# gau-nernst/llama-x

Measured on AMD Instinct MI355X. Metric: train tokens/sec Llama-3.1-8B seq4096 at 1/2/4/8 MI355X; p50 step ms, higher is better.
Workload: dtype bf16; 1 GPU; Llama-3.1-8B text-only LoRA r=16 bf16, seq=4096, 1 sequence per GPU, causal mask, base+LM head frozen (BASELINE.json configs[1]); random-init weights at 8B dimensions; seq_len=4096, parallelism=dp1, launch=hipGraph replay (fwd+bwd+AdamW), lm_head_rows=labelled only

## Files before the change

### include/llx.h

```cpp
#ifndef LLX_H
#define LLX_H

#include <stdint.h>

#ifdef __cplusplus
extern "C" {
#endif

typedef void* llx_stream_t;

int llx_version(void);
const char* llx_last_error_string(void);
int llx_device_info(int device, char* name, int len);

int llx_rmsnorm_fwd(const void* x, const void* w, void* y, float* rstd, int64_t rows, int64_t dim, float eps, llx_stream_t s);
int llx_rmsnorm_fwd_quant(const void* x, const void* w, void* y, float* rstd, void* q, int64_t ldq, void* qscale, int64_t rows, int64_t dim,
                          float eps, llx_stream_t s);
int64_t llx_rmsnorm_bwd_workspace_bytes(int64_t rows, int64_t dim);
int llx_rmsnorm_bwd(const void* dy, const void* x, const void* w, const float* rstd, void* dx, void* dw ,
                    int dw_accumulate, void* workspace, const void* dres ,
                    int64_t rows, int64_t dim, llx_stream_t s);

int llx_gemm_nt_bf16(const void* A, int64_t lda, const void* B, int64_t ldb, void* C, int64_t ldc, int64_t M, int64_t N, int64_t K,
                     const void* A2, int64_t lda2, const void* B2, int64_t ldb2, int64_t K2, int epilogue, const void* E, int64_t lde,
                     llx_stream_t s);
int llx_gemm_nt_bf16_rows(const void* A, int64_t lda, const void* B, int64_t ldb, void* C, int64_t ldc, int64_t M, int64_t N, int64_t K,
                          const void* A2, int64_t lda2, const void* B2, int64_t ldb2, int64_t K2, int epilogue, const void* E, int64_t lde,
                          const int32_t* m_valid, llx_stream_t s);
int llx_gemm_nt_bf16_splitk(const void* A, int64_t lda, const void* B, int64_t ldb, float* partial, int64_t M, int64_t N, int64_t K, int splits,
                            const int32_t* m_valid, llx_stream_t s);
int llx_splitk_combine(const float* partial, int splits, int64_t M, int64_t N, const int32_t* inv, const float* scale, void* out, int64_t ld_out,
                       llx_stream_t s);
int llx_gemm_nt_bf16_rope(const void* A, int64_t lda, const void* B, int64_t ldb, void* C, int64_t ldc, int64_t M, int64_t N, int64_t K,
                          const void* A2, int64_t lda2, const void* B2, int64_t ldb2, int64_t K2, const float* rope_table, int64_t rope_S,
                          int64_t rope_cols, llx_stream_t s);

int llx_gemm_tn_bf16(const void* A, int64_t lda, const void* B, int64_t ldb, void* C, int64_t ldc, int64_t M, int64_t N1, int64_t N2,
                     llx_stream_t s);
int llx_gemm_tn_bf16_rows(const void* A, int64_t lda, const void* B, int64_t ldb, void* C, int64_t ldc, int64_t M, int64_t N1, int64_t N2,
                          const int32_t* m_valid, llx_stream_t s);
// ... 135 lines not shown
```

### llama-x_amd/csrc/gemm_bf16.hip

```cpp
#include "common.h"
#include <type_traits>
#include <mutex>

#define BM 256
#define BN 256
#define BK 64
#define STAGE_BYTES (2 * 256 * BK * 2)
#define A_TILE_BYTES (256 * BK * 2)
#define EPI_ROW_BYTES 528
#define GEMM_LDS_BYTES (256 * EPI_ROW_BYTES)

enum { EPI_NONE = 0, EPI_RESIDUAL = 1, EPI_BIAS = 2, EPI_BIAS_GELU = 3, EPI_COLSCALE = 4, EPI_ROWCOLSCALE = 5, EPI_SWIGLU_BWD = 6, EPI_SWIGLU_FWD = 7, EPI_ROPE = 8, EPI_SPLITK = 9, EPI_ROWCOLSCALE_F32 = 10 };

struct GemmArgs {
  const bf16_t* A; const bf16_t* B; bf16_t* C;
  const bf16_t* A2; const bf16_t* B2;
  const bf16_t* E;
  const bf16_t* E2;
  int64_t lda, ldb, ldc, lde, lda2, ldb2;
  int M, N, K, K2;
  int grid_m, grid_n;
  int col0, col_end;
  const bf16_t* sa; const bf16_t* sb;
  const float* rope;
  int rope_S, rope_cols;
  const int* m_valid;
  float* C32;
  int splits;
};

typedef __attribute__((address_space(3))) void lds_void;
typedef const __attribute__((address_space(1))) void gbl_void;

__device__ __forceinline__ float gelu_erf(float x) { return 0.5f * x * (1.0f + erff(x * 0.70710678118654752440f)); }

template <int EPI, bool I8, int PIPE, int BNT = 256>
__global__ __launch_bounds__(512, 2) void gemm_nt_kernel(const GemmArgs g) {
  static_assert(BNT == 256 || BNT == 128, "tile width");
  static_assert(PIPE == 1, "the four-phase main loop is the only one");
  static_assert(BNT == 256 || EPI != EPI_SWIGLU_FWD, "the SwiGLU-forward epilogue needs the full tile");
  constexpr int ESZ = I8 ? 1 : 2;
  constexpr int TK = 128 / ESZ;
  constexpr int WNG = BNT / 64;
  constexpr int WR = 256 / (8 / WNG);
  constexpr int MI = WR / 16;
  constexpr int MH = MI / 2;
  constexpr int BSI = BNT / 64;
  constexpr int EROW = BNT * 2 + 16;
  extern __shared__ __attribute__((aligned(16))) char smem[];
  const int tid = threadIdx.x;
  const int lane = tid & 63;
  const int wave = __builtin_amdgcn_readfirstlane(tid >> 6);
  const int wm = wave / WNG, wn = wave % WNG;

  int grid_m = g.grid_m;
// ... 2 lines not shown
  const int nwg = grid_m * g.grid_n * nsplit;
  int bid = blockIdx.x;
  if (bid >= nwg) return;
  {
    const int q = nwg >> 3, r = nwg & 7, x = bid & 7;
    bid = (x < r ? x * (q + 1) : r * (q + 1) + (x - r) * q) + (bid >> 3);
  }
  const int split = EPI == EPI_SPLITK ? bid / (grid_m * g.grid_n) : 0;
  if constexpr (EPI == EPI_SPLITK) bid -= split * (grid_m * g.grid_n);
  const int GROUP_M = 4;
  const int width = GROUP_M * g.grid_n;
  const int group = bid / width;
  const int gsz = min(grid_m - group * GROUP_M, GROUP_M);
  const int pid_m = group * GROUP_M + ((bid % width) % gsz);
  const int pid_n = (bid % width) / gsz;
  constexpr bool SPLITN = EPI == EPI_SWIGLU_FWD;
  const int halfN = g.N >> 1;
  const int m0 = pid_m * BM, n0 = SPLITN ? pid_n * (BN / 2) : g.col0 + pid_n * BNT;
  auto col_of = [&](int nl) { return SPLITN ? (nl < BN / 2 ? n0 + nl : halfN + n0 + nl - BN / 2) : min(n0 + nl, g.col_end - 1); };

  const int srow = tid >> 3;
  const int schunk = (tid & 7) ^ ((tid >> 4) & 7);
  int arow[4], brow[4];
#pragma unroll
  for (int i = 0; i < 4; ++i) {
    arow[i] = min(m0 + i * 64 + srow, g.M - 1);
    brow[i] = SPLITN ? (i < 2 ? n0 + i * 64 + srow : halfN + n0 + (i - 2) * 64 + srow) : min(n0 + (i % BSI) * 64 + srow, g.col_end - 1);
  }
  const int nk1 = g.K / TK / nsplit;
  const int nk = nk1 + g.K2 / 64;
  const int kofs = split * nk1;
// ... 67 lines not shown
#pragma unroll
      for (int mi = 0; mi < MI; ++mi) rsv[mi] = bf2f(g.sa[min(m0 + wm * WR + mi * 16 + frow, g.M - 1)]);
#pragma unroll
      for (int mi = 0; mi < MI; ++mi) {
        const float rs = rsv[mi];
#pragma unroll
        for (int ni = 0; ni < 4; ++ni) {
          f32x4_t cf;
#pragma unroll
          for (int e = 0; e < 4; ++e) cf[e] = bf2f(f2bf(((float)acc[mi][ni][e] * rs) * sbv[ni][e]));
          acc[mi][ni] = __builtin_bit_cast(acc_t, cf);
        }
      }
    }
  };
  stage_q(0, 0); stage_q(0, 1); stage_q(0, 2); stage_q(0, 3);
  stage_q(1, 2); stage_q(1, 3); stage_q(1, 0);
  auto ktile = [&](int kt, auto ext_tag) __attribute__((always_inline)) {
    auto mfma = [&](const i32x4_t& b, const i32x4_t& a, acc_t& c) { mfma_t(ext_tag, b, a, c); };
    const char* sA = smem + (kt & 1) * STAGE_BYTES;
    const char* sB = sA + A_TILE_BYTES;
    if (kt + 1 < nk) {
      if constexpr (BSI == 4) asm volatile("s_waitcnt vmcnt(6)" ::: "memory");
      else asm volatile("s_waitcnt vmcnt(4)" ::: "memory");
    } else asm volatile("s_waitcnt vmcnt(0)" ::: "memory");
    __builtin_amdgcn_s_barrier();
    asm volatile("" ::: "memory");
    stage_q(kt + 1, 1);
    i32x4_t bfr[2][4], af[2 * MH];
#pragma unroll
// ... 154 lines not shown
          for (int e = 0; e < 4; ++e) c[e] = ((float)acc[mi][ni][e] * rs) * sbv[ni][e];
        }
      } else {
#pragma unroll
        for (int e = 0; e < 4; ++e) c[e] = acc[mi][ni][e];
      }
      u32x2_t pk;
      pk[0] = pack_bf2(c[0], c[1]);
      pk[1] = pack_bf2(c[2], c[3]);
      *reinterpret_cast<u32x2_t*>(smem + m * EROW + n * 2) = pk;
    }
  }
  __syncthreads();
  if constexpr (SPLITN) {
    bf16_t* H = const_cast<bf16_t*>(g.E);
#pragma unroll 4
    for (int it = 0; it < 8; ++it) {
      const int q = it * 512 + tid;
      const int row = q >> 4, cc = q & 15;
      const int gm = m0 + row, gn = n0 + cc * 8;
      if (gm < g.M) {
        const u32x4_t gv = *reinterpret_cast<const u32x4_t*>(smem + row * EPI_ROW_BYTES + cc * 16);
        const u32x4_t uv = *reinterpret_cast<const u32x4_t*>(smem + row * EPI_ROW_BYTES + (cc + 16) * 16);
        *reinterpret_cast<u32x4_t*>(g.C + (int64_t)gm * g.ldc + gn) = gv;
        *reinterpret_cast<u32x4_t*>(g.C + (int64_t)gm * g.ldc + halfN + gn) = uv;
        *reinterpret_cast<u32x4_t*>(H + (int64_t)gm * g.lde + gn) = swiglu_fwd8(gv, uv);
      }
    }
    return;
  }
  auto combine = [&](int it0, const u32x4_t (&aux0)[EB], const u32x4_t (&aux1)[EB]) {
#pragma unroll
    for (int j = 0; j < EB; ++j) {
      const int q = (it0 + j) * 512 + tid;
      const int row = q / (BNT / 8), cc = q % (BNT / 8);
      const int gm = m0 + row, gn = n0 + cc * 8;
      if (gm < g.M && gn < g.col_end) {
        u32x4_t v = *reinterpret_cast<const u32x4_t*>(smem + row * EROW + cc * 16);
        if constexpr (EPI == EPI_RESIDUAL) {
          const u32x4_t r = aux0[j];
#pragma unroll
// ... 40 lines not shown
  auto kern = gemm_nt_kernel<EPI, I8, 1, BNT>;
  static std::once_flag attr_once;
  static hipError_t attr_err = hipSuccess;
  std::call_once(attr_once, [&] { attr_err = hipFuncSetAttribute((const void*)kern, hipFuncAttributeMaxDynamicSharedMemorySize, GEMM_LDS_BYTES); });
  if (attr_err != hipSuccess) {
    llx_set_error("llx_gemm_nt_bf16: cannot raise dynamic LDS limit: %s", hipGetErrorString(attr_err));
    return LLX_ERR_LAUNCH;
  }
  hipLaunchKernelGGL(kern, dim3(a.grid_m * a.grid_n * (EPI == EPI_SPLITK ? a.splits : 1)), dim3(512), GEMM_LDS_BYTES, stream, a);
  LLX_LAUNCH_CHECK("llx_gemm_nt_bf16");
  return LLX_OK;
}

template <int EPI, bool I8 = false>
static int launch_gemm(const GemmArgs& a, hipStream_t stream) {
  if constexpr (EPI != EPI_SWIGLU_FWD) {
    const int tiles = a.grid_m * a.grid_n, tail = tiles % 256;
    if (a.col0 == 0 && a.col_end == a.N && a.N % 256 == 0 && tiles > 256 && tail > 0 && tail <= 128 && tail % a.grid_m == 0) {
      const int tail_cols = tail / a.grid_m * 256;
      GemmArgs full = a, half = a;
      full.col_end = a.N - tail_cols;
      full.grid_n = a.grid_n - tail / a.grid_m;
      half.col0 = a.N - tail_cols;
      half.grid_n = tail_cols / 128;
      const int rc = launch_gemm_p<EPI, I8, 256>(full, stream);
      if (rc != LLX_OK) return rc;
      return launch_gemm_p<EPI, I8, 128>(half, stream);
    }
  }
  return launch_gemm_p<EPI, I8>(a, stream);
}
// ... 6 lines not shown
  a.grid_m = (int)cdiv64(M, BM); a.grid_n = (int)cdiv64(N, BN);
  a.col_end = (int)N;
  a.splits = 1;
  return a;
}

static int check_extent(const char* who, int64_t M, int64_t N, int64_t K, int64_t lda, int64_t ldb, int esz) {
  LLX_REQUIRE(M < (1 << 30) && N < (1 << 30) && K < (1 << 30), "%s: dimension too large", who);
  LLX_REQUIRE(M * lda * esz < (int64_t)4294967296 && N * ldb * esz < (int64_t)4294967296, "%s: operand larger than 4 GiB (32-bit tile offsets)", who);
  return LLX_OK;
}

static int gemm_nt_bf16_impl(const void* A, int64_t lda, const void* B, int64_t ldb, void* C, int64_t ldc, int64_t M,
                             int64_t N, int64_t K, const void* A2, int64_t lda2, const void* B2, int64_t ldb2, int64_t K2,
                             int epilogue, const void* E, int64_t lde, const float* rope, int64_t rope_S, int64_t rope_cols,
                             hipStream_t stream, const int32_t* m_valid = nullptr) {
  LLX_REQUIRE(A && B && C, "llx_gemm_nt_bf16: null pointer");
  LLX_REQUIRE(M > 0 && N > 0 && K > 0, "llx_gemm_nt_bf16: empty problem M=%lld N=%lld K=%lld", (long long)M, (long long)N, (long long)K);
  LLX_REQUIRE(K % BK == 0 && K2 % BK == 0, "llx_gemm_nt_bf16: K=%lld and K2=%lld must be multiples of 64", (long long)K, (long long)K2);
  LLX_REQUIRE(N % 8 == 0, "llx_gemm_nt_bf16: N=%lld must be a multiple of 8", (long long)N);
  LLX_REQUIRE(lda % 8 == 0 && ldb % 8 == 0 && ldc % 8 == 0, "llx_gemm_nt_bf16: row strides must be multiples of 8 elements");
  LLX_REQUIRE(((uintptr_t)A | (uintptr_t)B | (uintptr_t)C) % 16 == 0, "llx_gemm_nt_bf16: pointers must be 16-byte aligned");
  LLX_REQUIRE(K2 == 0 || (A2 && B2 && lda2 % 8 == 0 && ldb2 % 8 == 0 && ((uintptr_t)A2 | (uintptr_t)B2) % 16 == 0),
              "llx_gemm_nt_bf16: bad K-extension operands");
  LLX_REQUIRE(epilogue == EPI_NONE || epilogue == EPI_ROPE || (E && (uintptr_t)E % 16 == 0), "llx_gemm_nt_bf16: epilogue operand missing/unaligned");
  LLX_REQUIRE(epilogue != EPI_ROPE || (rope && (uintptr_t)rope % 16 == 0 && rope_S > 0 && rope_cols >= 0 && rope_cols <= N && rope_cols % 128 == 0),
              "llx_gemm_nt_bf16_rope: need an aligned fp32 table, rope_S > 0 and rope_cols a multiple of 128 within N");
  LLX_REQUIRE((epilogue != EPI_RESIDUAL && epilogue != EPI_SWIGLU_BWD) || lde % 8 == 0, "llx_gemm_nt_bf16: residual / gate|up stride must be a multiple of 8");
  LLX_REQUIRE(epilogue != EPI_SWIGLU_BWD || (lde >= 2 * N && ldc >= 2 * N), "llx_gemm_nt_bf16: the SwiGLU-backward epilogue reads E[M,2N] (gate|up) and writes C[M,2N] (dg|du)");
  if (const int rc = check_extent("llx_gemm_nt_bf16", M, N, K, lda, ldb, 2); rc != LLX_OK) return rc;
  GemmArgs a = make_args(A, lda, B, ldb, C, ldc, M, N, K);
  a.A2 = (const bf16_t*)A2; a.B2 = (const bf16_t*)B2; a.lda2 = lda2; a.ldb2 = ldb2; a.K2 = (int)K2;
  a.E = (const bf16_t*)E; a.lde = lde;
  a.rope = rope; a.rope_S = (int)rope_S; a.rope_cols = (int)rope_cols;
  a.m_valid = m_valid;
  switch (epilogue) {
    case EPI_NONE: return launch_gemm<EPI_NONE>(a, stream);
    case EPI_RESIDUAL: return launch_gemm<EPI_RESIDUAL>(a, stream);
    case EPI_BIAS: return launch_gemm<EPI_BIAS>(a, stream);
    case EPI_BIAS_GELU: return launch_gemm<EPI_BIAS_GELU>(a, stream);
    case EPI_COLSCALE: return launch_gemm<EPI_COLSCALE>(a, stream);
    case EPI_SWIGLU_BWD: return launch_gemm<EPI_SWIGLU_BWD>(a, stream);
    case EPI_ROPE: return launch_gemm<EPI_ROPE>(a, stream);
    case EPI_SWIGLU_FWD:
      LLX_REQUIRE(N % 256 == 0 && lde % 8 == 0, "llx_gemm_nt_bf16: the SwiGLU-forward epilogue needs N = 2I with I a multiple of 128");
      a.grid_n = (int)(N / 256);
      return launch_gemm<EPI_SWIGLU_FWD>(a, stream);
    default: llx_set_error("llx_gemm_nt_bf16: unknown epilogue %d", epilogue); return LLX_ERR_UNSUPPORTED;
  }
}

extern "C" int llx_gemm_nt_bf16(const void* A, int64_t lda, const void* B, int64_t ldb, void* C, int64_t ldc, int64_t M,
                                int64_t N, int64_t K, const void* A2, int64_t lda2, const void* B2, int64_t ldb2, int64_t K2,
                                int epilogue, const void* E, int64_t lde, hipStream_t stream) {
  LLX_REQUIRE(epilogue != EPI_ROPE, "llx_gemm_nt_bf16: the RoPE epilogue is llx_gemm_nt_bf16_rope");
  return gemm_nt_bf16_impl(A, lda, B, ldb, C, ldc, M, N, K, A2, lda2, B2, ldb2, K2, epilogue, E, lde, nullptr, 0, 0, stream);
}

extern "C" int llx_gemm_nt_bf16_rows(const void* A, int64_t lda, const void* B, int64_t ldb, void* C, int64_t ldc, int64_t M,
                                     int64_t N, int64_t K, const void* A2, int64_t lda2, const void* B2, int64_t ldb2, int64_t K2,
                                     int epilogue, const void* E, int64_t lde, const int32_t* m_valid, hipStream_t stream) {
  LLX_REQUIRE(epilogue != EPI_ROPE, "llx_gemm_nt_bf16_rows: the RoPE epilogue is llx_gemm_nt_bf16_rope");
  LLX_REQUIRE(m_valid && (uintptr_t)m_valid % 4 == 0, "llx_gemm_nt_bf16_rows: m_valid must be a device int32 pointer");
  return gemm_nt_bf16_impl(A, lda, B, ldb, C, ldc, M, N, K, A2, lda2, B2, ldb2, K2, epilogue, E, lde, nullptr, 0, 0, stream, m_valid);
}

extern "C" int llx_gemm_nt_bf16_splitk(const void* A, int64_t lda, const void* B, int64_t ldb, float* partial, int64_t M, int64_t N,
                                       int64_t K, int splits, const int32_t* m_valid, hipStream_t stream) {
  LLX_REQUIRE(A && B && partial, "llx_gemm_nt_bf16_splitk: null pointer");
  LLX_REQUIRE(M > 0 && N > 0 && K > 0 && splits >= 1 && splits <= 16, "llx_gemm_nt_bf16_splitk: bad sizes");
  LLX_REQUIRE(K % ((int64_t)BK * splits) == 0, "llx_gemm_nt_bf16_splitk: K=%lld must be a multiple of 64 * splits (%d)", (long long)K, splits);
  LLX_REQUIRE(N % 8 == 0 && lda % 8 == 0 && ldb % 8 == 0, "llx_gemm_nt_bf16_splitk: N and the row strides must be multiples of 8");
  LLX_REQUIRE(((uintptr_t)A | (uintptr_t)B | (uintptr_t)partial) % 16 == 0, "llx_gemm_nt_bf16_splitk: pointers must be 16-byte aligned");
  if (const int rc = check_extent("llx_gemm_nt_bf16_splitk", M, N, K, lda, ldb, 2); rc != LLX_OK) return rc;
  LLX_REQUIRE(m_valid == nullptr || (uintptr_t)m_valid % 4 == 0, "llx_gemm_nt_bf16_splitk: m_valid must be a device int32 pointer");
  GemmArgs a = make_args(A, lda, B, ldb, nullptr, N, M, N, K);
  a.m_valid = m_valid;
  a.C32 = partial; a.splits = splits;
  return launch_gemm_p<EPI_SPLITK, false>(a, stream);
// ... 100 lines not shown
```

### llama-x_amd/csrc/skinny.hip

```cpp
#include "common.h"

typedef __attribute__((address_space(3))) s16x4_t lds_s16x4;
typedef __attribute__((ext_vector_type(8))) short s16x8_t;

#define SK_PAD 64

#define SNT_WAVES 8
#define SNT_UNROLL 8

struct SkinnyRanges { int lo[4], hi[4]; };

__device__ __forceinline__ void snt_scaled_store(const bf16x8_t& a, const bf16_t* cs, bf16_t* g) {
  const u32x4_t x = __builtin_bit_cast(u32x4_t, a);
  const u32x4_t c = *reinterpret_cast<const u32x4_t*>(cs);
  u32x4_t o;
#pragma unroll
  for (int e = 0; e < 4; ++e) o[e] = pack_bf2(bflo(x[e]) * bflo(c[e]), bfhi(x[e]) * bfhi(c[e]));
  *reinterpret_cast<u32x4_t*>(g) = o;
}

template <int NB, bool RANGED, bool SCALE = false>
__global__ __launch_bounds__(SNT_WAVES * 64) void skinny_nt_kernel(const bf16_t* __restrict__ X, int64_t ldx, const bf16_t* __restrict__ W,
                                                                   int64_t ldw, bf16_t* __restrict__ out, int M, int K, int R, SkinnyRanges kr,
                                                                   const bf16_t* __restrict__ cs = nullptr, bf16_t* __restrict__ G = nullptr,
// ... 420 lines not shown
    *reinterpret_cast<u32x2_t*>(out + (int64_t)(m0 + threadIdx.x) * SK_PAD + blockIdx.y * 4) = pk;
  }
}

extern "C" int llx_skinny_u_reduce(const void* upart, void* out, int64_t M, int64_t N, int64_t R, const int32_t* segs, int seg_count, hipStream_t stream) {
  LLX_REQUIRE(upart && out && M > 0 && N > 0 && R > 0 && R <= 64, "llx_skinny_u_reduce: bad arguments");
  TnSegs sg;
  int64_t total = 0;
  const int rc = tn_fill_segs(sg, segs, seg_count, N, R, &total);
  if (rc != LLX_OK) return rc;
  hipLaunchKernelGGL(skinny_u_reduce_kernel, dim3((unsigned)cdiv64(M, 64), SK_PAD / 4), dim3(256), 0, stream, (const float*)upart, (bf16_t*)out, (int)M, (int)R, sg);
  LLX_LAUNCH_CHECK("llx_skinny_u_reduce");
  return LLX_OK;
}

struct TnRed { const float* partial; bf16_t* out; int64_t out_ld, total; int nsplit, RP, R, N, transpose_out, accumulate, use_segs; float scale; TnSegs sg; };
struct TnRedMany { TnRed d[TN_MANY]; };

__global__ void skinny_tn_reduce_many_kernel(const TnRedMany m) {
  const TnRed& d = m.d[blockIdx.y];
  int64_t idx = (int64_t)blockIdx.x * blockDim.x + threadIdx.x;
  if (idx >= d.total) return;
  int r, n;
  bf16_t* dst;
  if (d.use_segs) {
    int s = 0;
    for (; s < d.sg.count; ++s) {
      const int64_t cnt = (int64_t)(d.sg.n_hi[s] - d.sg.n_lo[s]) * (d.sg.r_hi[s] - d.sg.r_lo[s]);
      if (idx < cnt) break;
      idx -= cnt;
// ... 193 lines not shown
```

### llama-x_amd/llx/_lib.py

```python
from __future__ import annotations

import ctypes
import os
from ctypes import c_char_p, c_float, c_int, c_int64, c_void_p

import torch

_HERE = os.path.dirname(os.path.abspath(__file__))
LIB_PATH = os.environ.get("LLX_LIB_PATH") or os.path.join(_HERE, "libllx_hip.so")

_lib = None

_P, _I, _L, _F = c_void_p, c_int, c_int64, c_float
SIGNATURES: dict[str, tuple] = {
    "llx_version": (c_int, []),
    "llx_last_error_string": (c_char_p, []),
    "llx_device_info": (c_int, [c_int, c_char_p, c_int]),
    "llx_rmsnorm_fwd": (c_int, [_P, _P, _P, _P, _L, _L, _F, _P]),
    "llx_rmsnorm_fwd_quant": (c_int, [_P, _P, _P, _P, _P, _L, _P, _L, _L, _F, _P]),
    "llx_rmsnorm_bwd_workspace_bytes": (c_int64, [_L, _L]),
    "llx_rmsnorm_bwd": (c_int, [_P, _P, _P, _P, _P, _P, _I, _P, _P, _L, _L, _P]),
    "llx_attn_flags_bytes": (c_int64, [_L, _L]),
    "llx_attn_tile_flags": (c_int, [_P, _P, _P, _L, _L, _P]),
    "llx_attn_fwd": (c_int, [_P, _L, _L, _P, _L, _L, _P, _L, _L, _P, _L, _L, _P, _P, _P, _P, _L, _L, _L, _L, _L, _F, _P]),
# ... 44 lines not shown
    "llx_gather_rows": (c_int, [_P, _L, _P, _P, _P, _L, _L, _L, _P]),
    "llx_scatter_rows": (c_int, [_P, _L, _P, _P, _P, _L, _L, _L, _P]),
    "llx_skinny_nt": (c_int, [_P, _L, _P, _L, _P, _L, _L, _L, _P, _P]),
    "llx_skinny_nt_scaled": (c_int, [_P, _L, _P, _L, _P, _L, _L, _L, _P, _P, _P, _L, _P]),
    "llx_rmsnorm_skinny_nt": (c_int, [_P, _P, _P, _L, _P, _P, _P, _L, _L, _L, _F, _P]),
    "llx_skinny_tn_workspace_bytes": (c_int64, [_L, _L, _L]),
    "llx_skinny_tn": (c_int, [_P, _P, _L, _P, _L, _L, _L, _L, _F, _I, _I, _P, _P, _I, _P]),
    "llx_skinny_tn_partial": (c_int, [_P, _P, _L, _L, _L, _L, _P, _P, _I, _P]),
    "llx_skinny_tn_partial_many": (c_int, [_I, _P, _P, _P, _P, _P, _P, _P, _P, _P, _P]),
    "llx_skinny_u_workspace_bytes": (_L, [_L, _L]),
    "llx_skinny_tn_partial_many_u": (c_int, [_I, _P, _P, _P, _P, _P, _P, _P, _P, _P, _P, _P, _P, _P]),
    "llx_skinny_u_reduce": (c_int, [_P, _P, _L, _L, _L, _P, _I, _P]),
    "llx_skinny_tn_partial_many_us": (c_int, [_I, _P, _P, _P, _P, _P, _P, _P, _P, _P, _P, _P, _P, _P, _P, _P, _P]),
    "llx_skinny_tn_reduce_many": (c_int, [_I, _P, _P, _P, _P, _P, _P, _P, _P, _P, _P, _P, _P]),
    "llx_gemm_nt_bf16": (c_int, [_P, _L, _P, _L, _P, _L, _L, _L, _L, _P, _L, _P, _L, _L, _I, _P, _L, _P]),
    "llx_gemm_nt_bf16_splitk": (c_int, [_P, _L, _P, _L, _P, _L, _L, _L, _I, _P, _P]),
    "llx_splitk_combine": (c_int, [_P, _I, _L, _L, _P, _P, _P, _L, _P]),
    "llx_gemm_nt_bf16_rows": (c_int, [_P, _L, _P, _L, _P, _L, _L, _L, _L, _P, _L, _P, _L, _L, _I, _P, _L, _P, _P]),
    "llx_gemm_tn_bf16": (c_int, [_P, _L, _P, _L, _P, _L, _L, _L, _L, _P]),
    "llx_gemm_tn_bf16_rows": (c_int, [_P, _L, _P, _L, _P, _L, _L, _L, _L, _P, _P]),
    "llx_gemm_nt_bf16_rope": (c_int, [_P, _L, _P, _L, _P, _L, _L, _L, _L, _P, _L, _P, _L, _L, _P, _L, _L, _P]),
}

DEBUG_SIGNATURES: dict[str, tuple] = {
    "llx_debug_attn_fwd_occupancy": (c_int, []),
    "llx_debug_attn_bwd_set_stamps": (c_int, [_P]),
    "llx_debug_attn_fwd_stamps": (c_int, [_P, _P, _P, _P, _L, _L, _L, _P, _P]),
}


# ... 48 lines not shown
```

### llama-x_amd/llx/kernels.py

```python
from __future__ import annotations

import ctypes
import math
import os
from dataclasses import dataclass
from typing import Optional, Sequence

import torch
from torch import Tensor

from . import _lib as L

BF16 = torch.bfloat16
EPI_NONE, EPI_RESIDUAL, EPI_BIAS, EPI_BIAS_GELU, EPI_COLSCALE = 0, 1, 2, 3, 4
EPI_SWIGLU_BWD = 6
EPI_SWIGLU_FWD = 7
SK_PAD = 64
GEMM_TRACE = None
ATTN_TRACE = None


def _lib():
    return L.load()

# ... 66 lines not shown
    dw = ws = None
    if need_dw:
        dw = dw_out if dw_out is not None else torch.empty(dim, device=x.device, dtype=BF16)
        assert dw.shape == (dim,) and dw.is_contiguous() and dw.dtype is BF16
        ws = torch.empty(_lib().llx_rmsnorm_bwd_workspace_bytes(rows, dim), device=x.device, dtype=torch.uint8)
    if dres is not None:
        dres = _rows2d(dres)
        assert dres.shape == x2.shape and dres.stride(0) == dim
    L.check(_lib().llx_rmsnorm_bwd(L.ptr(dy2), L.ptr(x2), L.ptr(w), L.ptr(rstd), L.ptr(dx), L.ptr(dw), 0, L.ptr(ws), L.ptr(dres), rows, dim,
                                   L.stream()), "llx_rmsnorm_bwd")
    return dx.view(x.shape), dw


def gemm_nt(a: Tensor, b: Tensor, *, out: Optional[Tensor] = None, a2: Optional[Tensor] = None, b2: Optional[Tensor] = None,
            epilogue: int = EPI_NONE, e: Optional[Tensor] = None, rope: Optional[tuple[Tensor, int, int]] = None,
            k2_eff: Optional[float] = None, m_valid: Optional[Tensor] = None, m_expect: Optional[float] = None) -> Tensor:
    _chk_bf16(a, b, a2, b2, e, out)
    assert a.dim() == 2 and b.dim() == 2 and a.shape[1] == b.shape[1], (a.shape, b.shape)
    assert a.stride(1) == 1 and b.stride(1) == 1
    M, K = a.shape
    N = b.shape[0]
    if epilogue == EPI_SWIGLU_BWD:
        assert out is not None and e is not None and out.shape == (M, 2 * N) and e.shape == (M, 2 * N) and out.stride(1) == 1 and e.stride(1) == 1
    else:
        if out is None:
            out = torch.empty(M, N, device=a.device, dtype=BF16)
        assert out.shape == (M, N) and out.stride(1) == 1
    K2 = 0
    if a2 is not None:
        assert b2 is not None and a2.shape[0] == M and b2.shape[0] == N and a2.shape[1] == b2.shape[1]
        assert a2.stride(1) == 1 and b2.stride(1) == 1
# ... 1 lines not shown
    lde = 0
    if epilogue == EPI_RESIDUAL:
        assert e is not None and e.shape == (M, N) and e.stride(1) == 1
        lde = e.stride(0)
    elif epilogue == EPI_SWIGLU_BWD:
        lde = e.stride(0)
    elif epilogue == EPI_SWIGLU_FWD:
        assert e is not None and N % 256 == 0 and e.shape == (M, N // 2) and e.stride(1) == 1
        lde = e.stride(0)
    elif epilogue != EPI_NONE:
        assert e is not None and e.shape == (N,) and e.is_contiguous()
    ev = None
    if GEMM_TRACE is not None:
        ev = (torch.cuda.Event(enable_timing=True), torch.cuda.Event(enable_timing=True))
        ev[0].record()
    if rope is not None:
        table, rs, rc = rope
        assert epilogue == EPI_NONE and table.dtype is torch.float32 and table.is_contiguous() and table.shape[0] >= rs and table.shape[1:] == (64, 2)
        L.check(_lib().llx_gemm_nt_bf16_rope(L.ptr(a), a.stride(0), L.ptr(b), b.stride(0), L.ptr(out), out.stride(0), M, N, K,
                                             L.ptr(a2), a2.stride(0) if a2 is not None else 0, L.ptr(b2), b2.stride(0) if b2 is not None else 0, K2,
                                             L.ptr(table), rs, rc, L.stream()), "llx_gemm_nt_bf16_rope")
    elif m_valid is not None:
        assert m_valid.dtype is torch.int32 and m_valid.numel() == 1 and m_valid.device == a.device
        L.check(_lib().llx_gemm_nt_bf16_rows(L.ptr(a), a.stride(0), L.ptr(b), b.stride(0), L.ptr(out), out.stride(0), M, N, K,
                                             L.ptr(a2), a2.stride(0) if a2 is not None else 0, L.ptr(b2), b2.stride(0) if b2 is not None else 0, K2,
                                             epilogue, L.ptr(e), lde, L.ptr(m_valid), L.stream()), "llx_gemm_nt_bf16_rows")
    else:
        L.check(_lib().llx_gemm_nt_bf16(L.ptr(a), a.stride(0), L.ptr(b), b.stride(0), L.ptr(out), out.stride(0), M, N, K,
                                        L.ptr(a2), a2.stride(0) if a2 is not None else 0, L.ptr(b2), b2.stride(0) if b2 is not None else 0, K2,
                                        epilogue, L.ptr(e), lde, L.stream()), "llx_gemm_nt_bf16")
    if ev is not None:
# ... 610 lines not shown
    assert x.dim() == 2 and w.dim() == 2 and x.shape[1] == w.shape[1] and x.stride(1) == 1 and w.stride(1) == 1
    M, K = x.shape
    R = w.shape[0]
    out = torch.empty(M, SK_PAD, device=x.device, dtype=BF16)
    kr = None
    if kranges is not None:
        assert len(kranges) == 8
        kr = (ctypes.c_int32 * 8)(*[int(v) for v in kranges])
    if colscale is not None:
        assert colscale.shape == (K,) and colscale.is_contiguous()
        g = torch.empty(M, K, device=x.device, dtype=BF16)
        L.check(_lib().llx_skinny_nt_scaled(L.ptr(x), x.stride(0), L.ptr(w), w.stride(0), L.ptr(out), M, K, R, kr, L.ptr(colscale), L.ptr(g), K,
                                            L.stream()), "llx_skinny_nt_scaled")
        return out, g
    L.check(_lib().llx_skinny_nt(L.ptr(x), x.stride(0), L.ptr(w), w.stride(0), L.ptr(out), M, K, R, kr, L.stream()), "llx_skinny_nt")
    return out


@dataclass
class TnQueued:
    ws: Tensor
    out: Tensor
    out_ld: int
    M: int
    N: int
    R: int
    scale: float
    transpose_out: int
    accumulate: int
    segs: Optional[ctypes.Array]
# ... 71 lines not shown
```

### llama-x_amd/llx/ops.py

```python
from __future__ import annotations

import os

from typing import Optional, Sequence

import torch
from torch import Tensor, nn
from torch.autograd import Function

from . import kernels as K
from ._lib import LlxError

BF16 = torch.bfloat16


def _cached_multi(tensors: Sequence[Tensor], tag: str, build):
    store = tensors[0].__dict__.setdefault("_llx_cache", {})
    key = tuple((t._version, str(t.device)) for t in tensors)
    hit = store.get(tag)
    if hit is not None and hit[0] == key:
        return hit[1]
    val = build()
    store[tag] = (key, val)
    return val
# ... 181 lines not shown
        if self.int8 and self.dynamic:
            return _cached_multi(ws, "cat_i8", lambda: torch.cat([w.detach() for w in ws], 0))
        if self.int8:
            return _cached_multi(ws, "cat_bf16", lambda: K.i8_to_bf16(torch.cat([w.detach() for w in ws], 0)))
        return _cached_multi(ws, "cat", lambda: torch.cat([w.detach() for w in ws], 0) if len(ws) > 1 else ws[0].detach())

    def wt_cat(self) -> Tensor:
        ws = self._weights()
        return _cached_multi(ws, "cat_t", lambda: K.transpose(torch.cat([w.detach() for w in ws], 0) if len(ws) > 1 else ws[0].detach()))

    def scale_cat(self) -> Tensor:
        ss = [m.weight.scale for m in self.members]
        return _cached_multi(ss, "cat_scale", lambda: torch.cat(ss, 0) if len(ss) > 1 else ss[0])

    def forward(self, x: Tensor, out: Optional[Tensor] = None, residual: Optional[Tensor] = None, swiglu_h: Optional[Tensor] = None,
                rope: Optional[tuple[Tensor, int, int]] = None, xq: Optional[tuple[Tensor, Tensor]] = None, t_pre: Optional[Tensor] = None):
        if out is None:
            out = torch.empty(x.shape[0], self.N, device=x.device, dtype=BF16)
        return out, self._forward(x, out, residual, swiglu_h, rope, xq, t_pre)

    def norm_can_make_t(self, dim: int) -> bool:
        return self.fused and self.R > 0 and self.packed is not None and K.rmsnorm_skinny_ok(dim)

    def wants_quantized_input(self) -> bool:
        return self.fused and self.int8 and self.dynamic

    def rope_fusable(self) -> bool:
        return self.fused and (not self.int8 or self.dynamic) and not self.dora

    def swiglu_fusable(self) -> bool:
        return self.fused and (not self.int8 or self.dynamic) and not self.dora and len(self.members) == 2 and self.Ns[0] % 128 == 0

    def _forward(self, x: Tensor, out: Tensor, residual: Optional[Tensor], swiglu_h: Optional[Tensor] = None,
                 rope: Optional[tuple[Tensor, int, int]] = None, xq: Optional[tuple[Tensor, Tensor]] = None, t_pre: Optional[Tensor] = None):
        if not self.fused:
            assert residual is None or len(self.members) == 1
            return [m.forward(x, out=out[:, o : o + n], residual=residual)[1] for m, o, n in zip(self.members, self.n_off, self.Ns)]
        t = b2 = None
        if self.R > 0:
            a_cat, b2, bT, a2t = self.packed or K.lora_group_pack([m.lora_a.detach() for m in self.members],
                                                                  [m.lora_b.detach() for m in self.members], self.K, self.scale)
            t = (t_pre if t_pre is not None else K.skinny_nt(x, a_cat), bT, a2t)
        if self.dora:
            assert swiglu_h is None and rope is None
            c, inv = dora_colscale(self.members, self.w_cat(), a_cat, b2)
            z = K.gemm_nt(x, self.w_cat(), a2=t[0], b2=b2, k2_eff=self.k2_fwd)
            K.scale(z, colscale=c, out=out)
            if residual is not None:
                K.add(out, residual, out=out)
            return (*t, z, c, inv)
        if not self.int8:
            if residual is not None:
                K.gemm_nt(x, self.w_cat(), out=out, a2=t[0] if t else None, b2=b2, epilogue=K.EPI_RESIDUAL, e=residual, k2_eff=self.k2_fwd)
            elif swiglu_h is not None:
                K.gemm_nt(x, self.w_cat(), out=out, a2=t[0] if t else None, b2=b2, epilogue=K.EPI_SWIGLU_FWD, e=swiglu_h, k2_eff=self.k2_fwd)
            else:
                K.gemm_nt(x, self.w_cat(), out=out, a2=t[0] if t else None, b2=b2, rope=rope, k2_eff=self.k2_fwd)
            return t
        if self.dynamic:
            from subclasses.int8 import quantize_int8_rowwise
            from subclasses.int8_mm import _launch as i8_gemm

            xi, xs = xq if xq is not None else quantize_int8_rowwise(x)
            a2, bb = (t[0], b2) if self.R > 0 else (None, None)
            if residual is not None:
                i8_gemm(xi, self.w_cat(), xs, self.scale_cat(), out=out, a2=a2, b2=bb, epilogue=K.EPI_RESIDUAL, e=residual)
            elif swiglu_h is not None:
                i8_gemm(xi, self.w_cat(), xs, self.scale_cat(), out=out, a2=a2, b2=bb, epilogue=K.EPI_SWIGLU_FWD, e=swiglu_h)
            else:
                i8_gemm(xi, self.w_cat(), xs, self.scale_cat(), out=out, a2=a2, b2=bb, rope=rope)
# ... 324 lines not shown
        return (dx.view(B, S, D) if (dx is not None and need_dx) else None, None, dnw, None, *g_qkv, *g_o)


_HEAD_COMPACT = os.environ.get("LLX_HEAD_COMPACT", "1") != "0"
_HEAD_SPLITK = max(1, int(os.environ.get("LLX_HEAD_SPLITK", "4")))
_HEAD_CHUNK_FORCED = "LLX_HEAD_CHUNK_ROWS" in os.environ
_HEAD_CHUNK_ROWS = max(256, int(os.environ.get("LLX_HEAD_CHUNK_ROWS", "8192")) // 256 * 256)


class MLPBlockMeta:
    def __init__(self, w13: GroupPlan, w2: GroupPlan, eps, fuse_norm, fuse_residual):
        self.w13, self.w2 = w13, w2
        self.eps, self.fuse_norm, self.fuse_residual = eps, fuse_norm, fuse_residual


class MLPBlockFn(Function):
    @staticmethod
    def forward(ctx, x: Tensor, norm_w: Optional[Tensor], meta: MLPBlockMeta, *tensors):
        K.L.require_cuda(x)
        shape = x.shape
        x2 = K._rows2d(x.contiguous())
        xn, rstd, xq, t_pre = _norm_prologue(meta, meta.w13, x2, norm_w)
        T, I = x2.shape[0], meta.w13.Ns[0]
        gu = torch.empty(T, 2 * I, device=x.device, dtype=BF16)
        if meta.w13.swiglu_fusable():
            h = torch.empty(T, I, device=x.device, dtype=BF16)
            _, t13 = meta.w13.forward(xn, gu, swiglu_h=h, xq=xq, t_pre=t_pre)
        else:
            _, t13 = meta.w13.forward(xn, gu, xq=xq, t_pre=t_pre)
            h = K.swiglu_fwd(gu[:, :I], gu[:, I:])
        y, t2 = meta.w2.forward(h, None, x2 if meta.fuse_residual else None)
        ctx.meta = meta
        _save(ctx, x, norm_w, x2, xn if meta.fuse_norm else None, rstd, gu, h, t13, t2)
        return y.view(shape)

    @staticmethod
    def backward(ctx, dy: Tensor):
        meta: MLPBlockMeta = ctx.meta
        x, norm_w, x2, xn, rstd, gu, h, t13, t2 = _load(ctx)
        if xn is None:
            xn = x2
        T, I = x2.shape[0], meta.w13.Ns[0]
        dy2 = K._rows2d(dy.contiguous())
        needs = list(ctx.needs_input_grad[3:])
        n_13 = len(meta.w13.tensors())
        n13, n2 = needs[:n_13], needs[n_13:]
# ... 114 lines not shown
```

Baseline: 30870 tokens/s.

## Fuse LoRA down-proj A-projection of SwiGLU output into gate/up GEMM epilogue

```diff
diff --git a/include/llx.h b/include/llx.h
--- a/include/llx.h
+++ b/include/llx.h
@@ -24,6 +24,11 @@
 int llx_gemm_nt_bf16(const void* A, int64_t lda, const void* B, int64_t ldb, void* C, int64_t ldc, int64_t M, int64_t N, int64_t K,
                      const void* A2, int64_t lda2, const void* B2, int64_t ldb2, int64_t K2, int epilogue, const void* E, int64_t lde,
                      llx_stream_t s);
+int llx_gemm_nt_bf16_swiglu_t(const void* A, int64_t lda, const void* B, int64_t ldb, void* C, int64_t ldc, int64_t M, int64_t N, int64_t K,
+                              const void* A2, int64_t lda2, const void* B2, int64_t ldb2, int64_t K2, void* H, int64_t ldh, const void* W,
+                              int64_t ldw, int64_t R, float* tpart, llx_stream_t s);
+int64_t llx_skinny_t_workspace_bytes(int64_t M, int64_t I, int64_t R);
+int llx_skinny_t_reduce(const void* tpart, void* out, int64_t M, int64_t R, int64_t ntiles, llx_stream_t s);
 int llx_gemm_nt_bf16_rows(const void* A, int64_t lda, const void* B, int64_t ldb, void* C, int64_t ldc, int64_t M, int64_t N, int64_t K,
                           const void* A2, int64_t lda2, const void* B2, int64_t ldb2, int64_t K2, int epilogue, const void* E, int64_t lde,
                           const int32_t* m_valid, llx_stream_t s);
diff --git a/llama-x_amd/csrc/gemm_bf16.hip b/llama-x_amd/csrc/gemm_bf16.hip
--- a/llama-x_amd/csrc/gemm_bf16.hip
+++ b/llama-x_amd/csrc/gemm_bf16.hip
@@ -10,7 +10,8 @@
 #define EPI_ROW_BYTES 528
 #define GEMM_LDS_BYTES (256 * EPI_ROW_BYTES)
 
-enum { EPI_NONE = 0, EPI_RESIDUAL = 1, EPI_BIAS = 2, EPI_BIAS_GELU = 3, EPI_COLSCALE = 4, EPI_ROWCOLSCALE = 5, EPI_SWIGLU_BWD = 6, EPI_SWIGLU_FWD = 7, EPI_ROPE = 8, EPI_SPLITK = 9, EPI_ROWCOLSCALE_F32 = 10 };
+enum { EPI_NONE = 0, EPI_RESIDUAL = 1, EPI_BIAS = 2, EPI_BIAS_GELU = 3, EPI_COLSCALE = 4, EPI_ROWCOLSCALE = 5, EPI_SWIGLU_BWD = 6, EPI_SWIGLU_FWD = 7, EPI_ROPE = 8, EPI_SPLITK = 9, EPI_ROWCOLSCALE_F32 = 10,
+       EPI_SWIGLU_FWD_T = 11 };
 
 struct GemmArgs {
   const bf16_t* A; const bf16_t* B; bf16_t* C;
@@ -27,6 +28,10 @@
   const int* m_valid;
   float* C32;
   int splits;
+  const bf16_t* tW;
+  int64_t ldtw;
+  float* tpart;
+  int tR;
 };
 
 typedef __attribute__((address_space(3))) void lds_void;
@@ -38,7 +43,7 @@
 __global__ __launch_bounds__(512, 2) void gemm_nt_kernel(const GemmArgs g) {
   static_assert(BNT == 256 || BNT == 128, "tile width");
   static_assert(PIPE == 1, "the four-phase main loop is the only one");
-  static_assert(BNT == 256 || EPI != EPI_SWIGLU_FWD, "the SwiGLU-forward epilogue needs the full tile");
+  static_assert(BNT == 256 || (EPI != EPI_SWIGLU_FWD && EPI != EPI_SWIGLU_FWD_T), "the SwiGLU-forward epilogue needs the full tile");
   constexpr int ESZ = I8 ? 1 : 2;
   constexpr int TK = 128 / ESZ;
   constexpr int WNG = BNT / 64;
@@ -71,7 +76,8 @@
   const int gsz = min(grid_m - group * GROUP_M, GROUP_M);
   const int pid_m = group * GROUP_M + ((bid % width) % gsz);
   const int pid_n = (bid % width) / gsz;
-  constexpr bool SPLITN = EPI == EPI_SWIGLU_FWD;
+  constexpr bool SPLITN = EPI == EPI_SWIGLU_FWD || EPI == EPI_SWIGLU_FWD_T;
+  constexpr bool TFUSE = EPI == EPI_SWIGLU_FWD_T;
   const int halfN = g.N >> 1;
   const int m0 = pid_m * BM, n0 = SPLITN ? pid_n * (BN / 2) : g.col0 + pid_n * BNT;
   auto col_of = [&](int nl) { return SPLITN ? (nl < BN / 2 ? n0 + nl : halfN + n0 + nl - BN / 2) : min(n0 + nl, g.col_end - 1); };
@@ -169,6 +175,13 @@
       }
     }
   };
+  bf16x8_t wf[4];
+  if constexpr (TFUSE) {
+    static_assert(!I8, "bf16 kernel only");
+    const bf16_t* wrow = g.tW + (int64_t)min(frow, g.tR - 1) * g.ldtw + n0 + fq * 8;
+#pragma unroll
+    for (int ks = 0; ks < 4; ++ks) wf[ks] = *reinterpret_cast<const bf16x8_t*>(wrow + ks * 32);
+  }
   stage_q(0, 0); stage_q(0, 1); stage_q(0, 2); stage_q(0, 3);
   stage_q(1, 2); stage_q(1, 3); stage_q(1, 0);
   auto ktile = [&](int kt, auto ext_tag) __attribute__((always_inline)) {
@@ -353,17 +366,41 @@
   __syncthreads();
   if constexpr (SPLITN) {
     bf16_t* H = const_cast<bf16_t*>(g.E);
+    if constexpr (TFUSE) {
+#pragma unroll
+      for (int ks = 0; ks < 4; ++ks) asm volatile("" : "+v"(wf[ks]));
+    }
 #pragma unroll 4
     for (int it = 0; it < 8; ++it) {
       const int q = it * 512 + tid;
-      const int row = q >> 4, cc = q & 15;
+      const int row = TFUSE ? wave * 32 + it * 4 + (lane >> 4) : q >> 4, cc = q & 15;
       const int gm = m0 + row, gn = n0 + cc * 8;
       if (gm < g.M) {
         const u32x4_t gv = *reinterpret_cast<const u32x4_t*>(smem + row * EPI_ROW_BYTES + cc * 16);
         const u32x4_t uv = *reinterpret_cast<const u32x4_t*>(smem + row * EPI_ROW_BYTES + (cc + 16) * 16);
         *reinterpret_cast<u32x4_t*>(g.C + (int64_t)gm * g.ldc + gn) = gv;
         *reinterpret_cast<u32x4_t*>(g.C + (int64_t)gm * g.ldc + halfN + gn) = uv;
-        *reinterpret_cast<u32x4_t*>(H + (int64_t)gm * g.lde + gn) = swiglu_fwd8(gv, uv);
+        const u32x4_t hv = swiglu_fwd8(gv, uv);
+        *reinterpret_cast<u32x4_t*>(H + (int64_t)gm * g.lde + gn) = hv;
+        if constexpr (TFUSE) *reinterpret_cast<u32x4_t*>(smem + row * EPI_ROW_BYTES + cc * 16) = hv;
+      }
+    }
+    if constexpr (TFUSE) {
+      asm volatile("s_waitcnt lgkmcnt(0)" ::: "memory");
+      __builtin_amdgcn_wave_barrier();
+#pragma unroll
+      for (int rf = 0; rf < 2; ++rf) {
+        const int rowl = (wave * 2 + rf) * 16 + frow;
+        const char* hrow = smem + rowl * EPI_ROW_BYTES + fq * 16;
+        f32x4_t t0 = {0.f, 0.f, 0.f, 0.f}, t1 = {0.f, 0.f, 0.f, 0.f};
+        t0 = __builtin_amdgcn_mfma_f32_16x16x32_bf16(wf[0], *reinterpret_cast<const bf16x8_t*>(hrow), t0, 0, 0, 0);
+        t1 = __builtin_amdgcn_mfma_f32_16x16x32_bf16(wf[1], *reinterpret_cast<const bf16x8_t*>(hrow + 64), t1, 0, 0, 0);
+        t0 = __builtin_amdgcn_mfma_f32_16x16x32_bf16(wf[2], *reinterpret_cast<const bf16x8_t*>(hrow + 128), t0, 0, 0, 0);
+        t1 = __builtin_amdgcn_mfma_f32_16x16x32_bf16(wf[3], *reinterpret_cast<const bf16x8_t*>(hrow + 192), t1, 0, 0, 0);
+        if (m0 + rowl < g.M) {
+#pragma unroll
+          for (int e = 0; e < 4; ++e) g.tpart[((int64_t)pid_n * 16 + fq * 4 + e) * g.M + m0 + rowl] = t0[e] + t1[e];
+        }
       }
     }
     return;
@@ -434,7 +471,7 @@
 
 template <int EPI, bool I8 = false>
 static int launch_gemm(const GemmArgs& a, hipStream_t stream) {
-  if constexpr (EPI != EPI_SWIGLU_FWD) {
+  if constexpr (EPI != EPI_SWIGLU_FWD && EPI != EPI_SWIGLU_FWD_T) {
     const int tiles = a.grid_m * a.grid_n, tail = tiles % 256;
     if (a.col0 == 0 && a.col_end == a.N && a.N % 256 == 0 && tiles > 256 && tail > 0 && tail <= 128 && tail % a.grid_m == 0) {
       const int tail_cols = tail / a.grid_m * 256;
@@ -471,7 +508,8 @@
 static int gemm_nt_bf16_impl(const void* A, int64_t lda, const void* B, int64_t ldb, void* C, int64_t ldc, int64_t M,
                              int64_t N, int64_t K, const void* A2, int64_t lda2, const void* B2, int64_t ldb2, int64_t K2,
                              int epilogue, const void* E, int64_t lde, const float* rope, int64_t rope_S, int64_t rope_cols,
-                             hipStream_t stream, const int32_t* m_valid = nullptr) {
+                             hipStream_t stream, const int32_t* m_valid = nullptr, const void* tW = nullptr, int64_t ldtw = 0,
+                             int64_t tR = 0, float* tpart = nullptr) {
   LLX_REQUIRE(A && B && C, "llx_gemm_nt_bf16: null pointer");
   LLX_REQUIRE(M > 0 && N > 0 && K > 0, "llx_gemm_nt_bf16: empty problem M=%lld N=%lld K=%lld", (long long)M, (long long)N, (long long)K);
   LLX_REQUIRE(K % BK == 0 && K2 % BK == 0, "llx_gemm_nt_bf16: K=%lld and K2=%lld must be multiples of 64", (long long)K, (long long)K2);
@@ -491,6 +529,7 @@
   a.E = (const bf16_t*)E; a.lde = lde;
   a.rope = rope; a.rope_S = (int)rope_S; a.rope_cols = (int)rope_cols;
   a.m_valid = m_valid;
+  a.tW = (const bf16_t*)tW; a.ldtw = ldtw; a.tR = (int)tR; a.tpart = tpart;
   switch (epilogue) {
     case EPI_NONE: return launch_gemm<EPI_NONE>(a, stream);
     case EPI_RESIDUAL: return launch_gemm<EPI_RESIDUAL>(a, stream);
@@ -502,6 +541,7 @@
     case EPI_SWIGLU_FWD:
       LLX_REQUIRE(N % 256 == 0 && lde % 8 == 0, "llx_gemm_nt_bf16: the SwiGLU-forward epilogue needs N = 2I with I a multiple of 128");
       a.grid_n = (int)(N / 256);
+      if (tpart != nullptr) return launch_gemm<EPI_SWIGLU_FWD_T>(a, stream);
       return launch_gemm<EPI_SWIGLU_FWD>(a, stream);
     default: llx_set_error("llx_gemm_nt_bf16: unknown epilogue %d", epilogue); return LLX_ERR_UNSUPPORTED;
   }
@@ -520,6 +560,14 @@
   LLX_REQUIRE(epilogue != EPI_ROPE, "llx_gemm_nt_bf16_rows: the RoPE epilogue is llx_gemm_nt_bf16_rope");
   LLX_REQUIRE(m_valid && (uintptr_t)m_valid % 4 == 0, "llx_gemm_nt_bf16_rows: m_valid must be a device int32 pointer");
   return gemm_nt_bf16_impl(A, lda, B, ldb, C, ldc, M, N, K, A2, lda2, B2, ldb2, K2, epilogue, E, lde, nullptr, 0, 0, stream, m_valid);
+}
+
+extern "C" int llx_gemm_nt_bf16_swiglu_t(const void* A, int64_t lda, const void* B, int64_t ldb, void* C, int64_t ldc, int64_t M, int64_t N,
+                                         int64_t K, const void* A2, int64_t lda2, const void* B2, int64_t ldb2, int64_t K2, void* H,
+                                         int64_t ldh, const void* W, int64_t ldw, int64_t R, float* tpart, hipStream_t stream) {
+  LLX_REQUIRE(W && tpart && R > 0 && R <= 16, "llx_gemm_nt_bf16_swiglu_t: need W, tpart and 0 < R <= 16 (R=%lld)", (long long)R);
+  LLX_REQUIRE(ldw % 8 == 0 && (uintptr_t)W % 16 == 0 && (uintptr_t)tpart % 16 == 0, "llx_gemm_nt_bf16_swiglu_t: W / tpart alignment");
+  return gemm_nt_bf16_impl(A, lda, B, ldb, C, ldc, M, N, K, A2, lda2, B2, ldb2, K2, EPI_SWIGLU_FWD, H, ldh, nullptr, 0, 0, stream, nullptr, W, ldw, R, tpart);
 }
 
 extern "C" int llx_gemm_nt_bf16_splitk(const void* A, int64_t lda, const void* B, int64_t ldb, float* partial, int64_t M, int64_t N,
diff --git a/llama-x_amd/csrc/skinny.hip b/llama-x_amd/csrc/skinny.hip
--- a/llama-x_amd/csrc/skinny.hip
+++ b/llama-x_amd/csrc/skinny.hip
@@ -458,6 +458,56 @@
   return LLX_OK;
 }
 
+#define TRD_SPLITS 4
+__global__ __launch_bounds__(256 * TRD_SPLITS) void skinny_t_reduce_kernel(const float* __restrict__ tpart, bf16_t* __restrict__ out, int M, int R, int RP,
+                                                                           int ntiles) {
+  __shared__ float tile[TRD_SPLITS][4][65];
+  const int m0 = blockIdx.x * 64, ml = threadIdx.x & 63, cl = (threadIdx.x >> 6) & 3, sp = threadIdx.x >> 8;
+  const int c = blockIdx.y * 4 + cl;
+  float sum = 0.f;
+  if (c < R) {
+    const int per = (ntiles + TRD_SPLITS - 1) / TRD_SPLITS;
+    const int t_lo = min(sp * per, ntiles), t_hi = min(t_lo + per, ntiles);
+    const int64_t stride = (int64_t)RP * M;
+    const float* src = tpart + (int64_t)c * M + min(m0 + ml, M - 1);
+    int t = t_lo;
+    for (; t + 8 <= t_hi; t += 8) {
+      float v[8];
+#pragma unroll
+      for (int j = 0; j < 8; ++j) v[j] = src[(t + j) * stride];
+#pragma unroll
+      for (int j = 0; j < 8; ++j) sum += v[j];
+    }
+    for (; t < t_hi; ++t) sum += src[t * stride];
+  }
+  tile[sp][cl][ml] = sum;
+  __syncthreads();
+  if (threadIdx.x < 64 && m0 + threadIdx.x < M) {
+    float v[4];
+#pragma unroll
+    for (int j = 0; j < 4; ++j) {
+      v[j] = tile[0][j][threadIdx.x];
+#pragma unroll
+      for (int s = 1; s < TRD_SPLITS; ++s) v[j] += tile[s][j][threadIdx.x];
+    }
+    u32x2_t pk;
+    pk[0] = pack_bf2(v[0], v[1]);
+    pk[1] = pack_bf2(v[2], v[3]);
+    *reinterpret_cast<u32x2_t*>(out + (int64_t)(m0 + threadIdx.x) * SK_PAD + blockIdx.y * 4) = pk;
+  }
+}
+
+extern "C" int64_t llx_skinny_t_workspace_bytes(int64_t M, int64_t I, int64_t R) { return cdiv64(I, 128) * cdiv64(R, 16) * 16 * M * 4; }
+
+extern "C" int llx_skinny_t_reduce(const void* tpart, void* out, int64_t M, int64_t R, int64_t ntiles, hipStream_t stream) {
+  LLX_REQUIRE(tpart && out && M > 0 && R > 0 && R <= 64 && ntiles > 0 && ntiles < (1 << 20), "llx_skinny_t_reduce: bad arguments");
+  LLX_REQUIRE((uintptr_t)out % 8 == 0, "llx_skinny_t_reduce: unaligned output");
+  hipLaunchKernelGGL(skinny_t_reduce_kernel, dim3((unsigned)cdiv64(M, 64), SK_PAD / 4), dim3(256 * TRD_SPLITS), 0, stream, (const float*)tpart, (bf16_t*)out,
+                     (int)M, (int)R, (int)cdiv64(R, 16) * 16, (int)ntiles);
+  LLX_LAUNCH_CHECK("llx_skinny_t_reduce");
+  return LLX_OK;
+}
+
 struct TnRed { const float* partial; bf16_t* out; int64_t out_ld, total; int nsplit, RP, R, N, transpose_out, accumulate, use_segs; float scale; TnSegs sg; };
 struct TnRedMany { TnRed d[TN_MANY]; };
 
diff --git a/llama-x_amd/llx/_lib.py b/llama-x_amd/llx/_lib.py
--- a/llama-x_amd/llx/_lib.py
+++ b/llama-x_amd/llx/_lib.py
@@ -82,6 +82,9 @@
     "llx_skinny_tn_partial_many_us": (c_int, [_I, _P, _P, _P, _P, _P, _P, _P, _P, _P, _P, _P, _P, _P, _P, _P, _P]),
     "llx_skinny_tn_reduce_many": (c_int, [_I, _P, _P, _P, _P, _P, _P, _P, _P, _P, _P, _P, _P]),
     "llx_gemm_nt_bf16": (c_int, [_P, _L, _P, _L, _P, _L, _L, _L, _L, _P, _L, _P, _L, _L, _I, _P, _L, _P]),
+    "llx_gemm_nt_bf16_swiglu_t": (c_int, [_P, _L, _P, _L, _P, _L, _L, _L, _L, _P, _L, _P, _L, _L, _P, _L, _P, _L, _L, _P, _P]),
+    "llx_skinny_t_workspace_bytes": (_L, [_L, _L, _L]),
+    "llx_skinny_t_reduce": (c_int, [_P, _P, _L, _L, _L, _P]),
     "llx_gemm_nt_bf16_splitk": (c_int, [_P, _L, _P, _L, _P, _L, _L, _L, _I, _P, _P]),
     "llx_splitk_combine": (c_int, [_P, _I, _L, _L, _P, _P, _P, _L, _P]),
     "llx_gemm_nt_bf16_rows": (c_int, [_P, _L, _P, _L, _P, _L, _L, _L, _L, _P, _L, _P, _L, _L, _I, _P, _L, _P, _P]),
diff --git a/llama-x_amd/llx/kernels.py b/llama-x_amd/llx/kernels.py
--- a/llama-x_amd/llx/kernels.py
+++ b/llama-x_amd/llx/kernels.py
@@ -104,7 +104,8 @@
 
 def gemm_nt(a: Tensor, b: Tensor, *, out: Optional[Tensor] = None, a2: Optional[Tensor] = None, b2: Optional[Tensor] = None,
             epilogue: int = EPI_NONE, e: Optional[Tensor] = None, rope: Optional[tuple[Tensor, int, int]] = None,
-            k2_eff: Optional[float] = None, m_valid: Optional[Tensor] = None, m_expect: Optional[float] = None) -> Tensor:
+            k2_eff: Optional[float] = None, m_valid: Optional[Tensor] = None, m_expect: Optional[float] = None,
+            t_from: Optional[tuple[Tensor, Tensor]] = None) -> Tensor:
     _chk_bf16(a, b, a2, b2, e, out)
     assert a.dim() == 2 and b.dim() == 2 and a.shape[1] == b.shape[1], (a.shape, b.shape)
     assert a.stride(1) == 1 and b.stride(1) == 1
@@ -136,7 +137,16 @@
     if GEMM_TRACE is not None:
         ev = (torch.cuda.Event(enable_timing=True), torch.cuda.Event(enable_timing=True))
         ev[0].record()
-    if rope is not None:
+    if t_from is not None:
+        tw, tpart = t_from
+        assert epilogue == EPI_SWIGLU_FWD and rope is None and m_valid is None
+        _chk_bf16(tw)
+        assert tw.dim() == 2 and tw.shape[1] == N // 2 and 0 < tw.shape[0] <= 16 and tw.stride(1) == 1
+        assert tpart.dtype is torch.float32 and tpart.is_contiguous() and tpart.numel() * 4 >= _lib().llx_skinny_t_workspace_bytes(M, N // 2, tw.shape[0])
+        L.check(_lib().llx_gemm_nt_bf16_swiglu_t(L.ptr(a), a.stride(0), L.ptr(b), b.stride(0), L.ptr(out), out.stride(0), M, N, K,
+                                                 L.ptr(a2), a2.stride(0) if a2 is not None else 0, L.ptr(b2), b2.stride(0) if b2 is not None else 0, K2,
+                                                 L.ptr(e), lde, L.ptr(tw), tw.stride(0), tw.shape[0], L.ptr(tpart), L.stream()), "llx_gemm_nt_bf16_swiglu_t")
+    elif rope is not None:
         table, rs, rc = rope
         assert epilogue == EPI_NONE and table.dtype is torch.float32 and table.is_contiguous() and table.shape[0] >= rs and table.shape[1:] == (64, 2)
         L.check(_lib().llx_gemm_nt_bf16_rope(L.ptr(a), a.stride(0), L.ptr(b), b.stride(0), L.ptr(out), out.stride(0), M, N, K,
@@ -777,6 +787,18 @@
                                             L.stream()), "llx_skinny_nt_scaled")
         return out, g
     L.check(_lib().llx_skinny_nt(L.ptr(x), x.stride(0), L.ptr(w), w.stride(0), L.ptr(out), M, K, R, kr, L.stream()), "llx_skinny_nt")
+    return out
+
+
+def skinny_t_workspace(M: int, I: int, R: int, device) -> Tensor:
+    return torch.empty(_lib().llx_skinny_t_workspace_bytes(M, I, R) // 4, device=device, dtype=torch.float32)
+
+
+def skinny_t_reduce(tpart: Tensor, M: int, I: int, R: int) -> Tensor:
+    assert tpart.dtype is torch.float32 and I % 128 == 0
+    L.require_cuda(tpart)
+    out = torch.empty(M, SK_PAD, device=tpart.device, dtype=BF16)
+    L.check(_lib().llx_skinny_t_reduce(L.ptr(tpart), L.ptr(out), M, R, I // 128, L.stream()), "llx_skinny_t_reduce")
     return out
 
 
diff --git a/llama-x_amd/llx/ops.py b/llama-x_amd/llx/ops.py
--- a/llama-x_amd/llx/ops.py
+++ b/llama-x_amd/llx/ops.py
@@ -219,10 +219,11 @@
         return _cached_multi(ss, "cat_scale", lambda: torch.cat(ss, 0) if len(ss) > 1 else ss[0])
 
     def forward(self, x: Tensor, out: Optional[Tensor] = None, residual: Optional[Tensor] = None, swiglu_h: Optional[Tensor] = None,
-                rope: Optional[tuple[Tensor, int, int]] = None, xq: Optional[tuple[Tensor, Tensor]] = None, t_pre: Optional[Tensor] = None):
+                rope: Optional[tuple[Tensor, int, int]] = None, xq: Optional[tuple[Tensor, Tensor]] = None, t_pre: Optional[Tensor] = None,
+                swiglu_t: Optional[tuple[Tensor, Tensor]] = None):
         if out is None:
             out = torch.empty(x.shape[0], self.N, device=x.device, dtype=BF16)
-        return out, self._forward(x, out, residual, swiglu_h, rope, xq, t_pre)
+        return out, self._forward(x, out, residual, swiglu_h, rope, xq, t_pre, swiglu_t)
 
     def norm_can_make_t(self, dim: int) -> bool:
         return self.fused and self.R > 0 and self.packed is not None and K.rmsnorm_skinny_ok(dim)
@@ -237,7 +238,9 @@
         return self.fused and (not self.int8 or self.dynamic) and not self.dora and len(self.members) == 2 and self.Ns[0] % 128 == 0
 
     def _forward(self, x: Tensor, out: Tensor, residual: Optional[Tensor], swiglu_h: Optional[Tensor] = None,
-                 rope: Optional[tuple[Tensor, int, int]] = None, xq: Optional[tuple[Tensor, Tensor]] = None, t_pre: Optional[Tensor] = None):
+                 rope: Optional[tuple[Tensor, int, int]] = None, xq: Optional[tuple[Tensor, Tensor]] = None, t_pre: Optional[Tensor] = None,
+                 swiglu_t: Optional[tuple[Tensor, Tensor]] = None):
+        assert swiglu_t is None or (swiglu_h is not None and self.fused and not self.int8 and not self.dora)
         if not self.fused:
             assert residual is None or len(self.members) == 1
             return [m.forward(x, out=out[:, o : o + n], residual=residual)[1] for m, o, n in zip(self.members, self.n_off, self.Ns)]
@@ -258,7 +261,8 @@
             if residual is not None:
                 K.gemm_nt(x, self.w_cat(), out=out, a2=t[0] if t else None, b2=b2, epilogue=K.EPI_RESIDUAL, e=residual, k2_eff=self.k2_fwd)
             elif swiglu_h is not None:
-                K.gemm_nt(x, self.w_cat(), out=out, a2=t[0] if t else None, b2=b2, epilogue=K.EPI_SWIGLU_FWD, e=swiglu_h, k2_eff=self.k2_fwd)
+                K.gemm_nt(x, self.w_cat(), out=out, a2=t[0] if t else None, b2=b2, epilogue=K.EPI_SWIGLU_FWD, e=swiglu_h, k2_eff=self.k2_fwd,
+                          t_from=swiglu_t)
             else:
                 K.gemm_nt(x, self.w_cat(), out=out, a2=t[0] if t else None, b2=b2, rope=rope, k2_eff=self.k2_fwd)
             return t
@@ -613,6 +617,12 @@
         self.eps, self.fuse_norm, self.fuse_residual = eps, fuse_norm, fuse_residual
 
 
+def _swiglu_makes_t2(meta: MLPBlockMeta) -> bool:
+    w13, w2 = meta.w13, meta.w2
+    return (w13.swiglu_fusable() and not w13.int8 and w2.fused and not w2.int8 and not w2.dora and len(w2.members) == 1
+            and 0 < w2.R <= 16 and w2.packed is not None and w2.K == w13.Ns[0])
+
+
 class MLPBlockFn(Function):
     @staticmethod
     def forward(ctx, x: Tensor, norm_w: Optional[Tensor], meta: MLPBlockMeta, *tensors):
@@ -622,13 +632,19 @@
         xn, rstd, xq, t_pre = _norm_prologue(meta, meta.w13, x2, norm_w)
         T, I = x2.shape[0], meta.w13.Ns[0]
         gu = torch.empty(T, 2 * I, device=x.device, dtype=BF16)
-        if meta.w13.swiglu_fusable():
+        t2_pre = None
+        if _swiglu_makes_t2(meta):
+            h = torch.empty(T, I, device=x.device, dtype=BF16)
+            tpart = K.skinny_t_workspace(T, I, meta.w2.R, x.device)
+            _, t13 = meta.w13.forward(xn, gu, swiglu_h=h, xq=xq, t_pre=t_pre, swiglu_t=(meta.w2.packed[0], tpart))
+            t2_pre = K.skinny_t_reduce(tpart, T, I, meta.w2.R)
+        elif meta.w13.swiglu_fusable():
             h = torch.empty(T, I, device=x.device, dtype=BF16)
             _, t13 = meta.w13.forward(xn, gu, swiglu_h=h, xq=xq, t_pre=t_pre)
         else:
             _, t13 = meta.w13.forward(xn, gu, xq=xq, t_pre=t_pre)
             h = K.swiglu_fwd(gu[:, :I], gu[:, I:])
-        y, t2 = meta.w2.forward(h, None, x2 if meta.fuse_residual else None)
+        y, t2 = meta.w2.forward(h, None, x2 if meta.fuse_residual else None, t_pre=t2_pre)
         ctx.meta = meta
         _save(ctx, x, norm_w, x2, xn if meta.fuse_norm else None, rstd, gu, h, t13, t2)
         return y.view(shape)
```

Result: no change. 30870 tokens/s (median of 4 runs) (-0.0%).
